# robertteleng/aria-slam

Hardware: AMD Instinct MI355X
Metric: frames/s ORB extract+BF-match, 640x480 @2000 kp (higher is better)
Workload: dtype u8

## Files before the change

### aria_slam_amd/csrc/orb_kernels.hip

```cpp
#include <hip/hip_runtime.h>

#include <cfloat>
#include <cstdint>
#include <cstdlib>

#include "common.h"
#include "orb_device.h"
#include "orb_kernels.h"

namespace aria {

struct PatternLaneMajor { uint32_t w[16][16]; };
constexpr PatternLaneMajor make_pattern_lane_major() {
    constexpr int src[1024] = {
#include "orb_pattern_31.inc"
    };
    PatternLaneMajor p{};
    for (int l = 0; l < 16; l++)
        for (int it = 0; it < 16; it++) {
            const int t = 16 * it + l;
            p.w[l][it] = ((uint32_t)(src[4 * t] & 0xFF)) | ((uint32_t)(src[4 * t + 1] & 0xFF) << 8) |
                         ((uint32_t)(src[4 * t + 2] & 0xFF) << 16) | ((uint32_t)(src[4 * t + 3] & 0xFF) << 24);
        }
    return p;
}
__device__ __attribute__((aligned(16))) const PatternLaneMajor kPattern31 = make_pattern_lane_major();

#define ARIA_UMAX_LIST {15, 15, 15, 15, 14, 14, 14, 13, 13, 12, 11, 10, 9, 8, 6, 3}

struct IcMaskLaneMajor { uint32_t m[16][16]; };
constexpr IcMaskLaneMajor make_ic_mask() {
    constexpr int umax[16] = ARIA_UMAX_LIST;
    IcMaskLaneMajor t{};
    for (int l = 0; l < 16; l++)
        for (int k = 0; k < 16; k++) {
            const int r = 2 * k + (l >> 3), j = l & 7;
            uint32_t w = 0;
            for (int b = 0; b < 4 && r < 31; b++) {
                const int u = 4 * j + b - 15, v = r - 15;
                const int au = u < 0 ? -u : u, av = v < 0 ? -v : v;
                if (au <= 15 && au <= umax[av]) w |= 0xFFu << (8 * b);
            }
            t.m[l][k] = w;
        }
    return t;
}
__device__ __attribute__((aligned(16))) const IcMaskLaneMajor kIcMask = make_ic_mask();

typedef short s2v __attribute__((ext_vector_type(2)));
__device__ __forceinline__ void harris_row_pairs(const uint8_t* rowp, int xs, int sh, bool dword_ok, uint32_t* E) {
    uint32_t w0, w1, w2;
    if (dword_ok) {
        const uint32_t* q = reinterpret_cast<const uint32_t*>(rowp + xs);
        w0 = q[0]; w1 = q[1]; w2 = q[2];
    } else {
        const uint8_t* q = rowp + xs;
        w0 = (uint32_t)q[0] | ((uint32_t)q[1] << 8) | ((uint32_t)q[2] << 16) | ((uint32_t)q[3] << 24);
        w1 = (uint32_t)q[4] | ((uint32_t)q[5] << 8) | ((uint32_t)q[6] << 16) | ((uint32_t)q[7] << 24);
        w2 = (uint32_t)q[8] | ((uint32_t)q[9] << 8) | ((uint32_t)q[10] << 16) | ((uint32_t)q[11] << 24);
    }
    const uint32_t a = __builtin_amdgcn_alignbyte(w1, w0, (uint32_t)sh);
    const uint32_t b = __builtin_amdgcn_alignbyte(w2, w1, (uint32_t)sh);
    E[0] = __builtin_amdgcn_perm(0u, a, 0x0c010c00u);
    E[1] = __builtin_amdgcn_perm(0u, a, 0x0c030c02u);
    E[2] = __builtin_amdgcn_perm(0u, b, 0x0c010c00u);
    E[3] = __builtin_amdgcn_perm(0u, b, 0x0c030c02u);
    E[4] = (w2 >> (8 * sh)) & 0xFFu;
}

__device__ __forceinline__ uint32_t pk16_add(uint32_t a, uint32_t b) {
    return __builtin_bit_cast(uint32_t, __builtin_bit_cast(s2v, a) + __builtin_bit_cast(s2v, b));
}
__device__ __forceinline__ uint32_t pk16_sub(uint32_t a, uint32_t b) {
    return __builtin_bit_cast(uint32_t, __builtin_bit_cast(s2v, a) - __builtin_bit_cast(s2v, b));
}

__device__ __forceinline__ float harris_response(const uint8_t* img, int pitch, int x, int y, bool dword_ok) {
    int a = 0, b = 0, c = 0;
    const int xs = (x - 4) & ~3, sh = (x - 4) & 3;
    const uint8_t* base = img + (int64_t)(y - 4) * pitch;
    uint32_t R[9][5];
#pragma unroll
    for (int r = 0; r < 9; r++) harris_row_pairs(base + (int64_t)r * pitch, xs, sh, dword_ok, R[r]);
#pragma unroll
    for (int i = 1; i <= 7; i++) {
        uint32_t sE[5], dE[5];
#pragma unroll
        for (int k = 0; k < 5; k++) {
            sE[k] = pk16_add(pk16_add(R[i - 1][k], R[i + 1][k]), pk16_add(R[i][k], R[i][k]));
            dE[k] = pk16_sub(R[i + 1][k], R[i - 1][k]);
        }
#pragma unroll
        for (int k = 0; k < 4; k++) {
            uint32_t ix = pk16_sub(sE[k + 1], sE[k]);
            const uint32_t dO = __builtin_amdgcn_alignbit(dE[k + 1], dE[k], 16);
            uint32_t iy = pk16_add(pk16_add(dE[k], dE[k + 1]), pk16_add(dO, dO));
            if (k == 3) { ix &= 0xFFFFu; iy &= 0xFFFFu; }
            const s2v vx = __builtin_bit_cast(s2v, ix), vy = __builtin_bit_cast(s2v, iy);
            a = __builtin_amdgcn_sdot2(vx, vx, a, false);
            b = __builtin_amdgcn_sdot2(vy, vy, b, false);
            c = __builtin_amdgcn_sdot2(vx, vy, c, false);
        }
    }
    const float scale = 1.f / ((1 << 2) * 7 * 255.f);
    const float scale_sq_sq = scale * scale * scale * scale;
    const float k = 0.04f;
    return ((float)a * (float)b - (float)c * (float)c - k * ((float)a + (float)b) * ((float)a + (float)b)) * scale_sq_sq;
}

__device__ void select_ovf_item(const Plan& P, const FrameSrc& S, const uint8_t* __restrict__ raw,
                                const uint32_t* __restrict__ cand, const int* __restrict__ cand_cnt,
                                uint4* __restrict__ sel, int* __restrict__ sel_cnt, int* __restrict__ err,
                                int* __restrict__ ovf, unsigned long long* __restrict__ keys, long long keys_cap,
                                uint4* __restrict__ osel, int osel_cap, int frame, int l, int* s_hist, int* s_misc);

template <bool INLINE_OVF, int NT>
__global__ __launch_bounds__(NT) void k_select(Plan P, FrameSrc S, const uint8_t* __restrict__ raw,
                                                const uint32_t* __restrict__ cand, const int* __restrict__ cand_cnt,
                                                uint4* __restrict__ sel, int* __restrict__ sel_cnt,
                                                int* __restrict__ err, unsigned long long* __restrict__ stamps,
                                                int* __restrict__ ovf, int2* __restrict__ ovf_items,
                                                unsigned long long* __restrict__ ovf_keys, long long ovf_keys_cap,
                                                uint4* __restrict__ osel, int osel_cap, int force_bitonic) {
    static_assert(kLevels == 8, "level rotation below assumes 8 levels");
    const int l = (int)((blockIdx.x + blockIdx.y) & 7u), frame = blockIdx.y;
#define SSTAMP(k) do { if (stamps && threadIdx.x == 0) stamps[((size_t)blockIdx.y * kLevels + l) * 8 + (k)] = __builtin_amdgcn_s_memtime(); } while (0)
    SSTAMP(0);
    extern __shared__ __attribute__((aligned(16))) unsigned long long s_keys[];
    __shared__ int s_hist[256];
    __shared__ int s_misc[4];
    __shared__ int s_wsum[NT / 64];
    __shared__ int s_bin[1024];

    const int tid = threadIdx.x;
    const bool lead = tid < 256;
    const LevelGeom g = P.lv[l];
    const uint32_t* clist = cand + (int64_t)frame * P.cand_frame_entries + g.cand_off;
    const int n = min(cand_cnt[frame * kLevels + l], g.cand_cap);
    const int q = g.quota;
    const int kSortCap = P.sort_cap;

    if (q == 0 || n == 0) {
        if (tid == 0) sel_cnt[frame * kLevels + l] = 0;
        return;
    }
    if (lead) s_hist[tid] = 0;
    if (tid == 0) { s_misc[1] = 0; s_misc[2] = 0; }
    __syncthreads();
    constexpr int kUnroll = 8;
    for (int i0 = 0; i0 < n; i0 += NT * kUnroll) {
        uint32_t v[kUnroll];
#pragma unroll
        for (int u = 0; u < kUnroll; u++) {
            const int i = i0 + u * NT + tid;
            v[u] = i < n ? clist[i] : 0u;
        }
#pragma unroll
        for (int u = 0; u < kUnroll; u++)
            if (i0 + u * NT + tid < n) atomicAdd(&s_hist[v[u] >> 22], 1);
    }
    __syncthreads();
    SSTAMP(1);
    {
        const int lane = tid & 63, wv = tid >> 6;
        int c = s_hist[255 - (tid & 255)];
#pragma unroll
        for (int d = 1; d < 64; d <<= 1) {
            const int o = __shfl_up(c, d);
            if (lane >= d) c += o;
        }
        if (lane == 63) s_wsum[wv] = c;
        if (tid == 0) s_misc[0] = 0;
        __syncthreads();
        int before = 0;
#pragma unroll
        for (int w = 0; w < 3; w++)
            if (w < wv) before += s_wsum[w];
        const int cum = c + before;
        const int own = s_hist[255 - (tid & 255)];
        if (lead && n > 2 * q && cum >= 2 * q && cum - own < 2 * q) s_misc[0] = 255 - tid;
        __syncthreads();
    }
    const int thr = s_misc[0];
    for (int i0 = 0; i0 < n; i0 += NT * kUnroll) {
        uint32_t v[kUnroll];
#pragma unroll
        for (int u = 0; u < kUnroll; u++) {
            const int i = i0 + u * NT + tid;
            v[u] = i < n ? clist[i] : 0u;
        }
#pragma unroll
        for (int u = 0; u < kUnroll; u++) {
            const bool keep = i0 + u * NT + tid < n && (int)(v[u] >> 22) >= thr;
            const unsigned long long m = __ballot(keep);
            if (m) {
                const int lane = tid & 63, leader = __ffsll((long long)m) - 1;
                int base = 0;
                if (lane == leader) base = atomicAdd(&s_misc[1], __popcll(m));
                base = __shfl(base, leader);
                const int slot = base + __popcll(m & ((1ull << lane) - 1ull));
                if (keep && slot < kSortCap) s_keys[slot] = (unsigned long long)v[u];
            }
        }
    }
    __syncthreads();
    SSTAMP(2);
    int pitch;
    const uint8_t* img = raw_level_ptr(P, S, raw, frame, l, pitch);
    {
        const int ns = min(s_misc[1], kSortCap);
        for (int i = tid; i < ns; i += NT) {
            const uint32_t cd = (uint32_t)s_keys[i];
            const int x = cd & 0x7FF, y = (cd >> 11) & 0x7FF;
            const float r = harris_response(img, pitch, x, y, (l > 0) || S.aligned4);
            uint32_t u = __float_as_uint(r);
            u = (u & 0x80000000u) ? ~u : (u | 0x80000000u);
            s_keys[i] = ((unsigned long long)(~u) << 32) | ((uint32_t)y << 16) | (uint32_t)x;
        }
    }
    __syncthreads();
    SSTAMP(3);
    int n1 = s_misc[1];
    if (n1 > kSortCap) {
        if (INLINE_OVF) {
            __shared__ __attribute__((aligned(8))) int s_ovm[8];
            if (!lead) return;
            select_ovf_item(P, S, raw, cand, cand_cnt, sel, sel_cnt, err, ovf, ovf_keys, ovf_keys_cap, osel, osel_cap, frame, l,
                            s_hist, s_ovm);
            return;
        }
        if (tid == 0) {
            sel_cnt[frame * kLevels + l] = 0;
            const int it = atomicAdd(&ovf[0], 1);
            if (it < kOvfItems) ovf_items[it] = make_int2(frame, l);
            else atomicOr(err, ERRBIT_SORT_OVERFLOW);
        }
        return;
    }
    __shared__ int s_srt[2];
    auto hbin = [](unsigned long long kk) { return (int)min((uint32_t)(kk >> 53), 1023u); };
    const bool cut = n1 > q + 64;
    for (int i = tid; i < 1024; i += NT) s_bin[i] = 0;
    if (tid == 0) { s_srt[0] = 1023; s_srt[1] = 0; }
    __syncthreads();
    for (int i = tid; i < n1; i += NT) atomicAdd(&s_bin[hbin(s_keys[i])], 1);
    __syncthreads();
    {
        const int lane = tid & 63, wv = tid >> 6;
        int b[4], tot = 0;
#pragma unroll
        for (int k = 0; k < 4; k++) { b[k] = lead ? s_bin[4 * tid + k] : 0; tot += b[k]; }
        int c = tot;
#pragma unroll
        for (int d = 1; d < 64; d <<= 1) {
            const int o = __shfl_up(c, d);
            if (lane >= d) c += o;
        }
        if (lane == 63) s_wsum[wv] = c;
        if (tid == 0) s_misc[1] = 0;
        __syncthreads();
        int run = c - tot;
#pragma unroll
        for (int w = 0; w < 3; w++)
            if (w < wv) run += s_wsum[w];
#pragma unroll
        for (int k = 0; k < 4; k++) {
            if (lead) s_bin[4 * tid + k] = run;
            if (lead && cut && run < q && run + b[k] >= q) s_srt[0] = 4 * tid + k;
            run += b[k];
        }
        __syncthreads();
        const int bc = s_srt[0];
        int mx = 0;
#pragma unroll
        for (int k = 0; k < 4; k++)
            if (lead && 4 * tid + k <= bc) mx = max(mx, b[k]);
        if (mx > 0) atomicMax(&s_srt[1], mx);
    }
    const int bcut = s_srt[0];
    if (cut) {
        for (int i0 = 0; i0 < n1; i0 += NT) {
            const int i = i0 + tid;
            const unsigned long long kk = i < n1 ? s_keys[i] : ~0ull;
            const bool keep = i < n1 && hbin(kk) <= bcut;
            __syncthreads();
            const unsigned long long m = __ballot(keep);
            if (m) {
                const int lane = tid & 63, leader = __ffsll((long long)m) - 1;
                int base = 0;
                if (lane == leader) base = atomicAdd(&s_misc[1], __popcll(m));
                base = __shfl(base, leader);
                if (keep) s_keys[base + __popcll(m & ((1ull << lane) - 1ull))] = kk;
            }
        }
        __syncthreads();
        n1 = s_misc[1];
    } else {
        __syncthreads();
    }
    const int upper = kSortCap >> 1;
    if (n1 <= upper && s_srt[1] <= 512 && !force_bitonic) {
        unsigned long long* s_up = s_keys + upper;
        for (int i = tid; i < n1; i += NT) {
            const unsigned long long kk = s_keys[i];
            s_up[atomicAdd(&s_bin[hbin(kk)], 1)] = kk;
        }
        __syncthreads();
        for (int i = tid; i < n1; i += NT) {
            const unsigned long long kk = s_up[i];
            const int b = hbin(kk);
            const int lo = b ? s_bin[b - 1] : 0, hi = s_bin[b];
            int r = lo;
            for (int j0 = lo; j0 < hi; j0 += 8) {
                unsigned long long o[8];
#pragma unroll
                for (int u = 0; u < 8; u++) o[u] = s_up[min(j0 + u, hi - 1)];
#pragma unroll
                for (int u = 0; u < 8; u++) r += (j0 + u < hi && o[u] < kk) ? 1 : 0;
            }
            s_keys[r] = kk;
        }
    } else {
        int np = 1;
        while (np < n1) np <<= 1;
        for (int i = n1 + tid; i < np; i += NT) s_keys[i] = ~0ull;
        __syncthreads();
        auto steps_of = [](int kk) { int n = 0; for (int jj = kk >> 1; jj > 0; jj >>= 1) n++; return n; };
        for (int k = 2; k <= np; k <<= 1) {
            int j = k >> 1;
            if (steps_of(k) & 1) {
                __syncthreads();
                for (int t0 = tid; t0 < (np >> 1); t0 += 2 * NT) {
                    const int ta = t0, tb = t0 + NT;
                    const bool hb = tb < (np >> 1);
                    const int a0 = ((ta & ~(j - 1)) << 1) | (ta & (j - 1)), a1 = a0 | j;
                    const int b0 = hb ? (((tb & ~(j - 1)) << 1) | (tb & (j - 1))) : a0, b1 = hb ? (b0 | j) : a1;
                    const unsigned long long xa = s_keys[a0], ya = s_keys[a1], xb = s_keys[b0], yb = s_keys[b1];
                    if ((xa > ya) == ((a0 & k) == 0)) { s_keys[a0] = ya; s_keys[a1] = xa; }
                    if (hb && (xb > yb) == ((b0 & k) == 0)) { s_keys[b0] = yb; s_keys[b1] = xb; }
                }
                __syncthreads();
                j >>= 1;
            }
            for (; j > 1; j >>= 2) {
                const int h = j >> 1;
                for (int t = tid; t < (np >> 2); t += NT) {
                    const int i = ((t & ~(h - 1)) << 2) | (t & (h - 1));
                    unsigned long long e0 = s_keys[i], e1 = s_keys[i + h], e2 = s_keys[i + j], e3 = s_keys[i + j + h];
                    const bool up = (i & k) == 0;
                    unsigned long long tmp;
                    if ((e0 > e2) == up) { tmp = e0; e0 = e2; e2 = tmp; }
                    if ((e1 > e3) == up) { tmp = e1; e1 = e3; e3 = tmp; }
                    if ((e0 > e1) == up) { tmp = e0; e0 = e1; e1 = tmp; }
                    if ((e2 > e3) == up) { tmp = e2; e2 = e3; e3 = tmp; }
                    s_keys[i] = e0; s_keys[i + h] = e1; s_keys[i + j] = e2; s_keys[i + j + h] = e3;
                }
                const int next_span = (j >> 2) > 1 ? 2 * (j >> 2) : ((k < np && !(steps_of(2 * k) & 1)) ? 2 * k : 0);
                if (2 * j > 256 || next_span > 256 || np > 4 * NT) __syncthreads();
                else { __threadfence_block(); __builtin_amdgcn_wave_barrier(); }
            }
        }
    }
    __syncthreads();
    SSTAMP(4);
    int n2 = n1;
    if (n1 > q) {
        const uint32_t cut = (uint32_t)(s_keys[q - 1] >> 32);
        for (int i = q + tid; i < n1; i += NT)
            if ((uint32_t)(s_keys[i] >> 32) == cut) atomicAdd(&s_misc[2], 1);
        __syncthreads();
        n2 = q + s_misc[2];
    }
    if (n2 > g.sel_cap) {
        if (INLINE_OVF) {
            __shared__ __attribute__((aligned(8))) int s_ovm[8];
            if (!lead) return;
            select_ovf_item(P, S, raw, cand, cand_cnt, sel, sel_cnt, err, ovf, ovf_keys, ovf_keys_cap, osel, osel_cap, frame, l,
                            s_hist, s_ovm);
            return;
        }
        if (tid == 0) {
            sel_cnt[frame * kLevels + l] = 0;
            const int it = atomicAdd(&ovf[0], 1);
            if (it < kOvfItems) ovf_items[it] = make_int2(frame, l);
            else atomicOr(err, ERRBIT_SEL_OVERFLOW);
        }
        return;
    }
    uint4* out = sel + (int64_t)frame * P.sel_frame_entries + g.sel_off;
    const int ts = (((g.w + 31) >> 5) * ((g.h + 31) >> 5) <= 1024) ? 5 : 6;
    const int tiles_x = (g.w + (1 << ts) - 1) >> ts, n_bins = tiles_x * ((g.h + (1 << ts) - 1) >> ts);
    for (int i = tid; i < n_bins; i += NT) s_bin[i] = 0;
    __syncthreads();
    for (int i = tid; i < n2; i += NT) {
        const uint32_t xy = (uint32_t)s_keys[i];
        atomicAdd(&s_bin[((xy >> (16 + ts)) * tiles_x) + ((xy & 0xFFFFu) >> ts)], 1);
    }
    __syncthreads();
    {
        const int lane = tid & 63, wv = tid >> 6;
        int b[4], tot = 0;
#pragma unroll
        for (int k = 0; k < 4; k++) { b[k] = (lead && 4 * tid + k < n_bins) ? s_bin[4 * tid + k] : 0; tot += b[k]; }
        int c = tot;
#pragma unroll
        for (int d = 1; d < 64; d <<= 1) {
            const int o = __shfl_up(c, d);
            if (lane >= d) c += o;
        }
        __syncthreads();
        if (lane == 63) s_wsum[wv] = c;
        __syncthreads();
        int run = c - tot;
#pragma unroll
        for (int w = 0; w < 3; w++)
            if (w < wv) run += s_wsum[w];
#pragma unroll
        for (int k = 0; k < 4; k++) {
            if (lead && 4 * tid + k < n_bins) s_bin[4 * tid + k] = run;
            run += b[k];
        }
    }
    __syncthreads();
    for (int i = tid; i < n2; i += NT) {
        const unsigned long long kk = s_keys[i];
        uint32_t u = ~(uint32_t)(kk >> 32);
        u = (u & 0x80000000u) ? (u & 0x7FFFFFFFu) : ~u;
        const uint32_t xy = (uint32_t)kk;
        const int pos = atomicAdd(&s_bin[((xy >> (16 + ts)) * tiles_x) + ((xy & 0xFFFFu) >> ts)], 1);
        out[pos] = make_uint4(xy, u, (uint32_t)i, 0u);
    }
    if (tid == 0) sel_cnt[frame * kLevels + l] = n2;
    SSTAMP(5);
#undef SSTAMP
}

__device__ __forceinline__ unsigned long long ovf_ld(const unsigned long long* p) {
    return __hip_atomic_load(p, __ATOMIC_RELAXED, __HIP_MEMORY_SCOPE_AGENT);
}
__device__ __forceinline__ void ovf_st(unsigned long long* p, unsigned long long v) {
    __hip_atomic_store(p, v, __ATOMIC_RELAXED, __HIP_MEMORY_SCOPE_AGENT);
}

__device__ __attribute__((noinline)) void select_ovf_item(const Plan& P, const FrameSrc& S, const uint8_t* __restrict__ raw,
                                const uint32_t* __restrict__ cand, const int* __restrict__ cand_cnt,
                                uint4* __restrict__ sel, int* __restrict__ sel_cnt, int* __restrict__ err,
                                int* __restrict__ ovf, unsigned long long* __restrict__ keys, long long keys_cap,
                                uint4* __restrict__ osel, int osel_cap, int frame, int l, int* s_hist, int* s_misc) {
    const int tid = threadIdx.x;
    {
        const LevelGeom g = P.lv[l];
        const uint32_t* clist = cand + (int64_t)frame * P.cand_frame_entries + g.cand_off;
        const int n = min(cand_cnt[frame * kLevels + l], g.cand_cap);
        const int q = g.quota;
        __syncthreads();
        s_hist[tid] = 0;
        if (tid < 8) s_misc[tid] = 0;
        __syncthreads();
        for (int i = tid; i < n; i += 256) atomicAdd(&s_hist[clist[i] >> 22], 1);
        __syncthreads();
        if (tid == 0) {
            int thr = 0, n1 = n;
            if (n > 2 * q) {
                int cum = 0;
                for (int sc = 255; sc >= 0; sc--) {
                    cum += s_hist[sc];
                    if (cum >= 2 * q) { thr = sc; n1 = cum; break; }
                }
            }
            long long np = 1;
            while (np < n1) np <<= 1;
            const long long base = (long long)atomicAdd(reinterpret_cast<unsigned long long*>(ovf + 2), (unsigned long long)np);
            s_misc[0] = thr;
            if (base + np > keys_cap) { atomicOr(err, ERRBIT_SORT_OVERFLOW); s_misc[3] = -1; }
            else { s_misc[3] = 0; }
            reinterpret_cast<long long*>(s_misc + 6)[0] = base;
            s_misc[5] = n1;
        }
        __syncthreads();
        if (s_misc[3] < 0) { if (tid == 0) sel_cnt[frame * kLevels + l] = 0; return; }
        const int thr = s_misc[0], n1 = s_misc[5];
        unsigned long long* K = keys + reinterpret_cast<long long*>(s_misc + 6)[0];
        long long np = 1;
        while (np < n1) np <<= 1;
        int pitch;
        const uint8_t* img = raw_level_ptr(P, S, raw, frame, l, pitch);
        for (int i0 = 0; i0 < n; i0 += 256) {
            const int i = i0 + tid;
            const uint32_t cd = i < n ? clist[i] : 0u;
            const bool keep = i < n && (int)(cd >> 22) >= thr;
            unsigned long long key = 0;
            if (keep) {
                const int x = cd & 0x7FF, y = (cd >> 11) & 0x7FF;
                const float r = harris_response(img, pitch, x, y, (l > 0) || S.aligned4);
                uint32_t u = __float_as_uint(r);
                u = (u & 0x80000000u) ? ~u : (u | 0x80000000u);
                key = ((unsigned long long)(~u) << 32) | ((uint32_t)y << 16) | (uint32_t)x;
            }
            const unsigned long long m = __ballot(keep);
            if (m) {
                const int lane = tid & 63, leader = __ffsll((long long)m) - 1;
                int base = 0;
                if (lane == leader) base = atomicAdd(&s_misc[1], __popcll(m));
                base = __shfl(base, leader);
                if (keep) ovf_st(&K[base + __popcll(m & ((1ull << lane) - 1ull))], key);
            }
        }
        for (long long i = n1 + tid; i < np; i += 256) ovf_st(&K[i], ~0ull);
        __syncthreads();
        for (long long k = 2; k <= np; k <<= 1)
            for (long long j = k >> 1; j > 0; j >>= 1) {
                for (long long t = tid; t < (np >> 1); t += 256) {
                    const long long a = ((t & ~(j - 1)) << 1) | (t & (j - 1)), b = a | j;
                    const unsigned long long xa = ovf_ld(&K[a]), xb = ovf_ld(&K[b]);
                    if ((xa > xb) == ((a & k) == 0)) { ovf_st(&K[a], xb); ovf_st(&K[b], xa); }
                }
                __syncthreads();
            }
        int n2 = n1;
        if (n1 > q) {
            const uint32_t cut = (uint32_t)(ovf_ld(&K[q - 1]) >> 32);
// ... 942 lines not shown
```

Before: 394,300.

## Batch Harris window loads across two keypoints and add occupancy launch bounds

Splits the Harris response into a window-load phase and a compute phase so each thread issues the loads for two candidate windows before computing either, hiding global memory latency. The aligned and unaligned paths are specialised at compile time. Candidate-list loads now clamp the index instead of branching, and the kernel gains a minimum-blocks-per-CU launch bound for the non-inline path. Keeping two windows in flight raises register pressure, and the launch bound may force spills.

```diff
diff --git a/aria_slam_amd/csrc/orb_kernels.hip b/aria_slam_amd/csrc/orb_kernels.hip
--- a/aria_slam_amd/csrc/orb_kernels.hip
+++ b/aria_slam_amd/csrc/orb_kernels.hip
@@ -48,24 +48,25 @@
 __device__ __attribute__((aligned(16))) const IcMaskLaneMajor kIcMask = make_ic_mask();
 
 typedef short s2v __attribute__((ext_vector_type(2)));
-__device__ __forceinline__ void harris_row_pairs(const uint8_t* rowp, int xs, int sh, bool dword_ok, uint32_t* E) {
-    uint32_t w0, w1, w2;
+__device__ __forceinline__ void harris_row_words(const uint8_t* rowp, uint32_t xs, bool dword_ok, uint32_t* w) {
     if (dword_ok) {
         const uint32_t* q = reinterpret_cast<const uint32_t*>(rowp + xs);
-        w0 = q[0]; w1 = q[1]; w2 = q[2];
+        w[0] = q[0]; w[1] = q[1]; w[2] = q[2];
     } else {
         const uint8_t* q = rowp + xs;
-        w0 = (uint32_t)q[0] | ((uint32_t)q[1] << 8) | ((uint32_t)q[2] << 16) | ((uint32_t)q[3] << 24);
-        w1 = (uint32_t)q[4] | ((uint32_t)q[5] << 8) | ((uint32_t)q[6] << 16) | ((uint32_t)q[7] << 24);
-        w2 = (uint32_t)q[8] | ((uint32_t)q[9] << 8) | ((uint32_t)q[10] << 16) | ((uint32_t)q[11] << 24);
-    }
-    const uint32_t a = __builtin_amdgcn_alignbyte(w1, w0, (uint32_t)sh);
-    const uint32_t b = __builtin_amdgcn_alignbyte(w2, w1, (uint32_t)sh);
+        w[0] = (uint32_t)q[0] | ((uint32_t)q[1] << 8) | ((uint32_t)q[2] << 16) | ((uint32_t)q[3] << 24);
+        w[1] = (uint32_t)q[4] | ((uint32_t)q[5] << 8) | ((uint32_t)q[6] << 16) | ((uint32_t)q[7] << 24);
+        w[2] = (uint32_t)q[8] | ((uint32_t)q[9] << 8) | ((uint32_t)q[10] << 16) | ((uint32_t)q[11] << 24);
+    }
+}
+__device__ __forceinline__ void harris_row_pairs(const uint32_t* w, int sh, uint32_t* E) {
+    const uint32_t a = __builtin_amdgcn_alignbyte(w[1], w[0], (uint32_t)sh);
+    const uint32_t b = __builtin_amdgcn_alignbyte(w[2], w[1], (uint32_t)sh);
     E[0] = __builtin_amdgcn_perm(0u, a, 0x0c010c00u);
     E[1] = __builtin_amdgcn_perm(0u, a, 0x0c030c02u);
     E[2] = __builtin_amdgcn_perm(0u, b, 0x0c010c00u);
     E[3] = __builtin_amdgcn_perm(0u, b, 0x0c030c02u);
-    E[4] = (w2 >> (8 * sh)) & 0xFFu;
+    E[4] = (w[2] >> (8 * sh)) & 0xFFu;
 }
 
 __device__ __forceinline__ uint32_t pk16_add(uint32_t a, uint32_t b) {
@@ -75,13 +76,17 @@
     return __builtin_bit_cast(uint32_t, __builtin_bit_cast(s2v, a) - __builtin_bit_cast(s2v, b));
 }
 
-__device__ __forceinline__ float harris_response(const uint8_t* img, int pitch, int x, int y, bool dword_ok) {
+__device__ __forceinline__ void harris_window(const uint8_t* img, int pitch, int x, int y, bool dword_ok, uint32_t* W) {
+    const uint32_t off = (uint32_t)((y - 4) * pitch + ((x - 4) & ~3));
+#pragma unroll
+    for (int r = 0; r < 9; r++) harris_row_words(img + (int64_t)r * pitch, off, dword_ok, W + 3 * r);
+}
+__device__ __forceinline__ float harris_from_window(const uint32_t* W, int x) {
     int a = 0, b = 0, c = 0;
-    const int xs = (x - 4) & ~3, sh = (x - 4) & 3;
-    const uint8_t* base = img + (int64_t)(y - 4) * pitch;
+    const int sh = (x - 4) & 3;
     uint32_t R[9][5];
 #pragma unroll
-    for (int r = 0; r < 9; r++) harris_row_pairs(base + (int64_t)r * pitch, xs, sh, dword_ok, R[r]);
+    for (int r = 0; r < 9; r++) harris_row_pairs(W + 3 * r, sh, R[r]);
 #pragma unroll
     for (int i = 1; i <= 7; i++) {
         uint32_t sE[5], dE[5];
@@ -107,6 +112,11 @@
     const float k = 0.04f;
     return ((float)a * (float)b - (float)c * (float)c - k * ((float)a + (float)b) * ((float)a + (float)b)) * scale_sq_sq;
 }
+__device__ __forceinline__ float harris_response(const uint8_t* img, int pitch, int x, int y, bool dword_ok) {
+    uint32_t W[27];
+    harris_window(img, pitch, x, y, dword_ok, W);
+    return harris_from_window(W, x);
+}
 
 __device__ void select_ovf_item(const Plan& P, const FrameSrc& S, const uint8_t* __restrict__ raw,
                                 const uint32_t* __restrict__ cand, const int* __restrict__ cand_cnt,
@@ -114,8 +124,26 @@
                                 int* __restrict__ ovf, unsigned long long* __restrict__ keys, long long keys_cap,
                                 uint4* __restrict__ osel, int osel_cap, int frame, int l, int* s_hist, int* s_misc);
 
+template <int WIN, int NT, bool DWORD_OK>
+__device__ __forceinline__ void harris_keys(unsigned long long* s_keys, int ns, const uint8_t* img, int pitch) {
+    for (int i0 = threadIdx.x; i0 < ns; i0 += NT * WIN) {
+        uint32_t cd[WIN], W[WIN][27];
+#pragma unroll
+        for (int h = 0; h < WIN; h++) cd[h] = (uint32_t)s_keys[i0 + h * NT < ns ? i0 + h * NT : i0];
+#pragma unroll
+        for (int h = 0; h < WIN; h++) harris_window(img, pitch, cd[h] & 0x7FF, (cd[h] >> 11) & 0x7FF, DWORD_OK, W[h]);
+#pragma unroll
+        for (int h = 0; h < WIN; h++) {
+            const int x = cd[h] & 0x7FF, y = (cd[h] >> 11) & 0x7FF;
+            uint32_t u = __float_as_uint(harris_from_window(W[h], x));
+            u = (u & 0x80000000u) ? ~u : (u | 0x80000000u);
+            if (i0 + h * NT < ns) s_keys[i0 + h * NT] = ((unsigned long long)(~u) << 32) | ((uint32_t)y << 16) | (uint32_t)x;
+        }
+    }
+}
+
 template <bool INLINE_OVF, int NT>
-__global__ __launch_bounds__(NT) void k_select(Plan P, FrameSrc S, const uint8_t* __restrict__ raw,
+__global__ __launch_bounds__(NT, INLINE_OVF ? 1 : 4) void k_select(Plan P, FrameSrc S, const uint8_t* __restrict__ raw,
                                                 const uint32_t* __restrict__ cand, const int* __restrict__ cand_cnt,
                                                 uint4* __restrict__ sel, int* __restrict__ sel_cnt,
                                                 int* __restrict__ err, unsigned long long* __restrict__ stamps,
@@ -151,10 +179,7 @@
     for (int i0 = 0; i0 < n; i0 += NT * kUnroll) {
         uint32_t v[kUnroll];
 #pragma unroll
-        for (int u = 0; u < kUnroll; u++) {
-            const int i = i0 + u * NT + tid;
-            v[u] = i < n ? clist[i] : 0u;
-        }
+        for (int u = 0; u < kUnroll; u++) v[u] = clist[min(i0 + u * NT + tid, n - 1)];
 #pragma unroll
         for (int u = 0; u < kUnroll; u++)
             if (i0 + u * NT + tid < n) atomicAdd(&s_hist[v[u] >> 22], 1);
@@ -185,10 +210,7 @@
     for (int i0 = 0; i0 < n; i0 += NT * kUnroll) {
         uint32_t v[kUnroll];
 #pragma unroll
-        for (int u = 0; u < kUnroll; u++) {
-            const int i = i0 + u * NT + tid;
-            v[u] = i < n ? clist[i] : 0u;
-        }
+        for (int u = 0; u < kUnroll; u++) v[u] = clist[min(i0 + u * NT + tid, n - 1)];
 #pragma unroll
         for (int u = 0; u < kUnroll; u++) {
             const bool keep = i0 + u * NT + tid < n && (int)(v[u] >> 22) >= thr;
@@ -209,14 +231,8 @@
     const uint8_t* img = raw_level_ptr(P, S, raw, frame, l, pitch);
     {
         const int ns = min(s_misc[1], kSortCap);
-        for (int i = tid; i < ns; i += NT) {
-            const uint32_t cd = (uint32_t)s_keys[i];
-            const int x = cd & 0x7FF, y = (cd >> 11) & 0x7FF;
-            const float r = harris_response(img, pitch, x, y, (l > 0) || S.aligned4);
-            uint32_t u = __float_as_uint(r);
-            u = (u & 0x80000000u) ? ~u : (u | 0x80000000u);
-            s_keys[i] = ((unsigned long long)(~u) << 32) | ((uint32_t)y << 16) | (uint32_t)x;
-        }
+        if ((l > 0) || S.aligned4) harris_keys<2, NT, true>(s_keys, ns, img, pitch);
+        else harris_keys<1, NT, false>(s_keys, ns, img, pitch);
     }
     __syncthreads();
     SSTAMP(3);
```

Result: no change. 390,100, median of 3 (-1.0%).
